# 10XGenomics/vartrix

Hardware: NVIDIA H100
Metric: reads_sw_scored_per_sec (higher is better)
Workload: dtype int16x2

## Files before the change

vartrix_b200/csrc/vtx_sw_fold.cuh:

```cuda
#pragma once
#include <cuda/atomic>
#include "vtx_sw.cuh"
#include "vtx_fold_ring.cuh"

namespace vtx {

constexpr int kFoldP = 96;
constexpr int kFoldC1 = 12;
constexpr int kFoldPPW = 4;
constexpr int kFoldR = 19;
constexpr int kFoldMaxRead = 8 * kFoldR;
constexpr int kFoldMaxMid = 40;
constexpr int kFoldRows = kFoldMaxRead + 4;
constexpr int kFoldCodeStride = kFoldMaxRead + 16;
constexpr int kFoldPairRows = 25;
#ifndef VTX_FOLD_UNROLL
#define VTX_FOLD_UNROLL 4
#endif
constexpr int kFoldDeepWarps = 20, kFoldDeepSlots = 9;
constexpr int kFoldShallowWarps = 13;
#ifndef VTX_FOLD_DEEP_DEPTH
#define VTX_FOLD_DEEP_DEPTH 6
#endif
constexpr uint32_t kFoldDeepDepth = VTX_FOLD_DEEP_DEPTH;
constexpr int kFoldUnroll = VTX_FOLD_UNROLL;
#ifndef VTX_FOLD_MID_UNROLL
#define VTX_FOLD_MID_UNROLL 1
#endif
constexpr int kFoldMidUnroll = VTX_FOLD_MID_UNROLL;

constexpr size_t kFoldSlotBytes = (size_t(kFoldPairRows) * kFoldP + size_t(kFoldMaxMid) * 8) * 4;
constexpr size_t kFoldWarpBytes = size_t(kFoldPPW) * kFoldRows * 8 + 32 + size_t(2 * kFoldPPW) * kFoldCodeStride;
static_assert(kFoldSlotBytes % 16 == 0 && kFoldWarpBytes % 16 == 0, "slots and warp areas stay 16-byte aligned");
template <int S> __host__ __device__ constexpr size_t fold_ring_bytes() { return (sizeof(FoldRing<S>) + 15) & ~size_t(15); }
template <int W, int S> __host__ __device__ constexpr size_t fold_cta_bytes()
{
    return fold_ring_bytes<S>() + S * kFoldSlotBytes + W * kFoldWarpBytes;
}

struct FoldSyncDev {
    using ref = cuda::atomic_ref<uint32_t, cuda::thread_scope_block>;
    __device__ static bool try_lock(uint32_t* p)
    {
        uint32_t z = 0;
        return ref(*p).compare_exchange_strong(z, 1u, cuda::memory_order_acquire, cuda::memory_order_relaxed);
    }
    __device__ static void unlock(uint32_t* p) { ref(*p).store(0u, cuda::memory_order_release); }
    __device__ static uint32_t grab(uint32_t* cursor) { return atomicAdd(cursor, 1u); }
    __device__ static uint32_t load_relaxed(uint32_t* p) { return ref(*p).load(cuda::memory_order_relaxed); }
    __device__ static uint32_t load_acquire(uint32_t* p) { return ref(*p).load(cuda::memory_order_acquire); }
    __device__ static void store_relaxed(uint32_t* p, uint32_t v) { ref(*p).store(v, cuda::memory_order_relaxed); }
    __device__ static void store_release(uint32_t* p, uint32_t v) { ref(*p).store(v, cuda::memory_order_release); }
    __device__ static void add(uint32_t* p, uint32_t v) { ref(*p).fetch_add(v, cuda::memory_order_relaxed); }
    __device__ static void sub_release(uint32_t* p, uint32_t v) { ref(*p).fetch_sub(v, cuda::memory_order_release); }
    __device__ static void pause() { __nanosleep(100); }
};

__device__ __forceinline__ uint32_t fold_locate(const uint32_t* __restrict__ ts, uint32_t n, uint32_t lo, uint32_t t,
                                                int lane)
{
    uint32_t hi = n, step = 1;
    for (;;) {
        const uint32_t i = lo + uint32_t(lane + 1) * step;
        const uint32_t k = __popc(__ballot_sync(0xffffffffu, i < hi && __ldg(ts + i) <= t));
        lo += k * step;
        if (k < 32) hi = min(hi, lo + step);
        if (hi - lo <= 1) return lo;
        step = (hi - lo + 31) / 32;
    }
}

constexpr int kJuncH = -2 * kGoe - kBias, kJuncE = -kGapOpen - kBias;
constexpr uint32_t kJuncH2 = (uint32_t(uint16_t(int16_t(kJuncH - 1))) << 16) | uint32_t(uint16_t(int16_t(kJuncH)));
constexpr uint32_t kJuncE2 = (uint32_t(uint16_t(int16_t(kJuncE - 1))) << 16) | uint32_t(uint16_t(int16_t(kJuncE)));

static_assert(kGapExtend < 0 && kGapOpen <= 0, "the vertical gap is a running maximum only if go <= 0");
constexpr uint32_t kFoldRowY2 = uint32_t(-kGapExtend) * 0x10001u;
constexpr uint32_t kGO2 = pack2(kGapOpen, kGapOpen);
constexpr uint32_t kScanNeg2 = pack2(kBias - 1024, kBias - 1024);
__host__ __device__ constexpr uint32_t fold_row_hg_add(int c)
{
    return (uint32_t(uint16_t(int16_t(kGoe + c * kGapExtend - 1))) << 16) | uint32_t(uint16_t(int16_t(kGoe + c * kGapExtend)));
}
static_assert(fold_row_hg_add(0) == kGoeAdd, "row 0 adds plain goe");

template <int W, int S, bool SHARED>
__global__ void __launch_bounds__(W * 32, 1) vtx_k_sw_fold(const SwArgs a)
{
    constexpr int C1 = kFoldC1, P = kFoldP, R = kFoldR, M = 8;
    constexpr int RS1 = P;

    extern __shared__ __align__(16) uint8_t smem_raw[];
    const int lane = threadIdx.x & 31, warp = threadIdx.x >> 5;
    const int u = lane >> 3, g = lane & 7;
    FoldRing<S>& ring = *reinterpret_cast<FoldRing<S>*>(smem_raw);
    uint8_t* const slots = smem_raw + fold_ring_bytes<S>();
    uint2* bnd = reinterpret_cast<uint2*>(slots + S * kFoldSlotBytes + warp * kFoldWarpBytes);
    uint8_t* codes = reinterpret_cast<uint8_t*>(bnd + kFoldPPW * kFoldRows + 4);

    const uint32_t n_tiles = __ldg(a.tile_start + a.n_loci);
    static_assert(SHARED || S == W, "per-warp tables: one slot per warp");
    const uint32_t run_len = SHARED ? fold_run_len(n_tiles, gridDim.x, W, kTileChunk)
                                    : max(1u, min(uint32_t(kTileChunk), n_tiles / (gridDim.x * W * 16u)));
    const uint32_t one = a.one;
    uint32_t w_next = 0, w_end = 0, w_locus = 0, w_cached = kFoldNoTile;
    if (threadIdx.x == 0) ring_init(ring);
    __syncthreads();

    for (;;) {
        __syncwarp();
        uint32_t tile, locus, slot;
        bool build;
        if constexpr (SHARED) {
            FoldTake tk{};
            if (lane == 0) tk = ring_take<FoldSyncDev>(ring, a.tile_counter, run_len, n_tiles);
            tile = __shfl_sync(0xffffffffu, tk.tile, 0);
            if (tile == kFoldNoTile) break;
            locus = fold_locate(a.tile_start, a.n_loci, __shfl_sync(0xffffffffu, tk.hint, 0), tile, lane);
            FoldBook bk{};
            if (lane == 0) bk = ring_book<FoldSyncDev>(ring, tk.ticket, locus);
            slot = __shfl_sync(0xffffffffu, bk.slot, 0);
            build = __shfl_sync(0xffffffffu, bk.build, 0);
        } else {
            if (w_next == w_end) {
                uint32_t chunk = 0;
                if (lane == 0) chunk = atomicAdd(a.tile_counter, 1u);
                chunk = __shfl_sync(0xffffffffu, chunk, 0);
                w_next = chunk * run_len;
                if (w_next >= n_tiles) break;
                w_end = min(w_next + run_len, n_tiles);
                w_locus = upper_locus(a.tile_start, a.n_loci, w_next);
            }
            tile = w_next++;
            while (tile >= __ldg(a.tile_start + w_locus + 1)) ++w_locus;
            locus = w_locus;
            slot = warp;
            build = locus != w_cached;
            w_cached = locus;
        }
        const uint32_t p0 = __ldg(a.pair_start + locus) + kFoldPPW * (tile - __ldg(a.tile_start + locus));
        const uint32_t p_end = __ldg(a.pair_start + locus + 1);
        uint32_t* prof = reinterpret_cast<uint32_t*>(slots + slot * kFoldSlotBytes);
        uint32_t* midtab = prof + kFoldPairRows * RS1;
        if (build) {
            const uint8_t* rh = a.hap_bytes + __ldg(a.ref_off + locus);
            const uint8_t* ah = a.hap_bytes + __ldg(a.alt_off + locus);
            const int n_ref = int(__ldg(a.ref_len + locus)), n_alt = int(__ldg(a.alt_len + locus));
            const int mid_ref = n_ref - 2 * P, mid_alt = n_alt - 2 * P;
            if (lane == 0) ring.mids[slot] = uint32_t(mid_ref) | uint32_t(mid_alt) << 16;
            if (lane < P / 4) {
                uint32_t fb[4], sb[4];
#pragma unroll
                for (int k = 0; k < 4; ++k) {
                    fb[k] = hap_code(__ldg(rh + 4 * lane + k));
                    sb[k] = hap_code(__ldg(rh + (n_ref - 1 - 4 * lane - k)));
                }
#pragma unroll
                for (uint32_t ra = 0; ra < 5; ++ra)
#pragma unroll
                    for (uint32_t rb = 0; rb < 5; ++rb) {
                        uint32_t w[4];
#pragma unroll
                        for (int k = 0; k < 4; ++k)
                            w[k] = pack2(ra == fb[k] ? kProfMatch : kProfMis, rb == sb[k] ? kProfMatch : kProfMis);
                        reinterpret_cast<uint4*>(prof + (5 * ra + rb) * RS1)[lane] = make_uint4(w[0], w[1], w[2], w[3]);
                    }
            }
            const int lmax = max(mid_ref, mid_alt);
            for (int idx = lane; idx < lmax * 8; idx += 32) {
                const int k = idx >> 3;
                const uint32_t r = uint32_t(idx & 7);
                const uint32_t rb = k < mid_ref ? hap_code(__ldg(rh + P + k)) : 5u;
                const uint32_t ab = k < mid_alt ? hap_code(__ldg(ah + P + k)) : 5u;
                midtab[idx] = pack2(r == rb ? kProfMatch : kProfMis, r == ab ? kProfMatch : kProfMis);
            }
            __syncwarp();
            if (SHARED && lane == 0) ring_publish<FoldSyncDev>(ring, slot);
        } else if (SHARED) {
            ring_wait<FoldSyncDev>(ring, slot);
        }
        const int mid_ref = int(ring.mids[slot] & 0xFFFFu), mid_alt = int(ring.mids[slot] >> 16);
        const uint32_t pair = p0 + u;
        const bool active = pair < p_end;
        int m = 0;
        uint8_t* cf = codes + (2 * u) * kFoldCodeStride;
        uint8_t* cp = cf + kFoldCodeStride;
        {
            const uint8_t* nib = nullptr;
            if (active) {
                const uint32_t rd = __ldg(a.pair_read + pair);
                m = int(__ldg(a.read_len + rd));
                nib = a.read_nib + __ldg(a.read_off + rd);
            }
            for (int e = g; e < kFoldCodeStride; e += 8)
                if (e < M || e >= M + m) cf[e] = 4;
            for (int b = g; 2 * b < m; b += 8) {
                const uint32_t by = __ldg(nib + b);
                cf[M + 2 * b] = uint8_t(nib_code(by >> 4));
                if (2 * b + 1 < m) cf[M + 2 * b + 1] = uint8_t(nib_code(by & 0xF));
            }
            __syncwarp();
            for (int e = g; e < kFoldCodeStride; e += 8)
                cp[e] = (e < M || e >= M + m) ? uint8_t(5 * 4 + 4) : uint8_t(5 * cf[e] + cf[2 * M + m - 1 - e]);
        }
        int mmax = m;
#pragma unroll
        for (int o = 16; o >= 1; o >>= 1) mmax = max(mmax, __shfl_xor_sync(0xffffffffu, mmax, o));
        __syncwarp();

        uint2* my_bnd = bnd + u * kFoldRows;
        const uint2* row_bnd = my_bnd + 7;
        uint32_t best;
        {
            uint32_t hg[C1], f[C1];
#pragma unroll
            for (int c = 0; c < C1; ++c) { hg[c] = kGOE2; f[c] = kNEG2; }
            uint32_t hg_last = kGOE2, e_last = kNEG2, diag_save = kGOE2;
            best = kBIAS2;
            const uint8_t* cA = cp + M - g;
            const uint32_t* lane_p = prof + g * C1;
            const int steps = mmax + 7;
#pragma unroll kFoldUnroll
            for (int t = 0; t < steps; ++t) {
                uint32_t hl = __shfl_up_sync(0xffffffffu, hg_last, 1, 8);
                uint32_t el = __shfl_up_sync(0xffffffffu, e_last, 1, 8);
                if (g == 0) { hl = kGOE2; el = kNEG2; }
                const uint4* pa = reinterpret_cast<const uint4*>(lane_p + uint32_t(cA[t]) * RS1);
                uint32_t diag = diag_save;
                diag_save = hl;
                uint32_t e = el, eg = hl, hleft = hl;
#pragma unroll
                for (int q = 0; q < C1 / 4; ++q) {
                    const uint4 a4 = pa[q];
                    const uint32_t sv[4] = { a4.x, a4.y, a4.z, a4.w };
                    uint32_t hh[4];
#pragma unroll
                    for (int k = 0; k < 4; ++k) {
                        const int c = 4 * q + k;
                        const uint32_t fc = __viaddmax_s16x2(f[c], kGE2, hg[c]);
                        e = __viaddmax_s16x2(e, kGE2, eg);
                        const uint32_t h = sw_h(diag, one, sv[k], fc, e);
                        hh[k] = h;
                        diag = hg[c];
                        hleft = hadd(h, one, c);
                        eg = hleft;
                        hg[c] = hleft;
                        f[c] = fc;
                    }
                    best = __vimax3_s16x2(best, hh[0], hh[1]);
                    best = __vimax3_s16x2(best, hh[2], hh[3]);
                }
                hg_last = hleft;
                e_last = e;
                if (g == 7) my_bnd[t] = make_uint2(hleft, e);
            }
#pragma unroll
            for (int o = 4; o >= 1; o >>= 1) best = __vmaxs2(best, __shfl_xor_sync(0xffffffffu, best, o));
            best = __vmaxs2(best, __byte_perm(best, 0, 0x1032));
        }
        __syncwarp();

        {
            const int lmax = max(mid_ref, mid_alt), lmin = min(mid_ref, mid_alt);
            const uint32_t short_mask = mid_ref < mid_alt ? 0x0000FFFFu : mid_alt < mid_ref ? 0xFFFF0000u : 0u;
            const int k_short = lmin != lmax ? lmin - 1 : -1;
            uint32_t hg[R], e[R], rc[R];
            const uint8_t* cfm = cf + M + R * g;
#pragma unroll
            for (int c = 0; c < R; ++c) {
                const int row = R * g + c;
                uint2 b = make_uint2(kGOE2, kNEG2);
                if (row < mmax) b = row_bnd[row];
                hg[c] = __byte_perm(b.x, 0, 0x1010);
                e[c] = __byte_perm(b.y, 0, 0x1010);
                rc[c] = uint32_t(cfm[c]) * 4u;
            }
            const int jlim = m - 2 - R * g;
            const uint2* jbnd = row_bnd + jlim;
            auto junction = [&](uint32_t mask) {
                uint32_t cross = kBIAS2;
#pragma unroll
                for (int c = 0; c < R; ++c) {
                    uint2 b = make_uint2(kGOE2, kGOE2);
                    if (c <= jlim) b = jbnd[-c];
                    const uint32_t ph = __byte_perm(b.x, 0, 0x3232), pe = __byte_perm(b.y, 0, 0x3232);
                    const uint32_t x1 = hg[c] + ph + kJuncH2;
                    const uint32_t x2 = e[c] + pe + kJuncE2;
                    cross = __vimax3_s16x2(cross, x1, x2);
                }
                best = __vmaxs2(best, (cross & mask) | (kBIAS2 & ~mask));
            };
            const uint8_t* tab = reinterpret_cast<const uint8_t*>(midtab);
#pragma unroll kFoldMidUnroll
            for (int k = 0; k < lmax; ++k) {
                const uint8_t* trow = tab + 32 * k;
                uint32_t diag = __shfl_up_sync(0xffffffffu, hg[R - 1], 1, 8);
                if (g == 0) diag = kGOE2;
                uint32_t aa[2], yy[2], ymax = kBIAS2;
#pragma unroll
                for (int c = 0; c < R; ++c) {
                    const uint32_t sv = *reinterpret_cast<const uint32_t*>(trow + rc[c]);
                    const uint32_t ec = __viaddmax_s16x2(e[c], kGE2, hg[c]);
                    const uint32_t av = __vimax3_s16x2(diag + sv, ec, kBIAS2);
                    const uint32_t yv = av + kFoldRowY2 * uint32_t(c);
                    diag = hg[c];
                    hg[c] = yv;
                    e[c] = ec;
                    aa[c & 1] = av;
                    yy[c & 1] = yv;
                    if (c & 1) {
                        best = __vimax3_s16x2(best, aa[0], aa[1]);
                        ymax = __vimax3_s16x2(ymax, yy[0], yy[1]);
                    }
                }
                if (R & 1) {
                    best = __vmaxs2(best, aa[0]);
                    ymax = __vmaxs2(ymax, yy[0]);
                }
                const uint32_t lane_ofs = uint32_t(-kGapExtend * R * g) * 0x10001u;
                uint32_t p = __shfl_up_sync(0xffffffffu, ymax + lane_ofs, 1, 8);
                if (g == 0) p = kScanNeg2;
#pragma unroll
                for (int o = 1; o < 8; o <<= 1) p = __vmaxs2(p, __shfl_up_sync(0xffffffffu, p, o, 8));
                p -= lane_ofs;
#pragma unroll
                for (int c = 0; c < R; ++c) {
                    const uint32_t yv = hg[c];
                    hg[c] = __viaddmax_s16x2(p, kGO2, yv) + fold_row_hg_add(c);
                    if (c + 1 < R) p = __vmaxs2(p, yv);
                }
                if (k == k_short) junction(short_mask);
            }
            junction(~short_mask);
#pragma unroll
            for (int o = 4; o >= 1; o >>= 1) best = __vmaxs2(best, __shfl_xor_sync(0xffffffffu, best, o));
            __syncwarp();
            if (SHARED && lane == 0) ring_release<FoldSyncDev>(ring, slot);
            if (active && g == 0) call_and_scatter(a, pair, best - kBIAS2);
        }
    }
}

}
```

Baseline: 169.5 million.

## Extend fold through shared mid-haplotype prefix before splitting ref/alt lanes

Detects how many middle haplotype bases ref and alt share at both ends and builds per-column 25-entry pair profiles for them. The kernel then runs those shared columns in a fused forward/backward mode before switching into the existing ref/alt split, shortening the split loop and junction span. The intent is to reduce the per-read column work in the middle region, at the cost of extra build logic, a parked boundary write to shared memory, and a repacked mids encoding limited to 8-bit lengths.

```diff
diff --git a/vartrix_b200/csrc/vtx_sw_fold.cuh b/vartrix_b200/csrc/vtx_sw_fold.cuh
--- a/vartrix_b200/csrc/vtx_sw_fold.cuh
+++ b/vartrix_b200/csrc/vtx_sw_fold.cuh
@@ -29,7 +29,8 @@
 #endif
 constexpr int kFoldMidUnroll = VTX_FOLD_MID_UNROLL;
 
-constexpr size_t kFoldSlotBytes = (size_t(kFoldPairRows) * kFoldP + size_t(kFoldMaxMid) * 8) * 4;
+constexpr int kFoldMidTabBytes = kFoldMaxMid * 32, kFoldExtColBytes = kFoldPairRows * 4;
+constexpr size_t kFoldSlotBytes = size_t(kFoldPairRows) * kFoldP * 4 + kFoldMidTabBytes;
 constexpr size_t kFoldWarpBytes = size_t(kFoldPPW) * kFoldRows * 8 + 32 + size_t(2 * kFoldPPW) * kFoldCodeStride;
 static_assert(kFoldSlotBytes % 16 == 0 && kFoldWarpBytes % 16 == 0, "slots and warp areas stay 16-byte aligned");
 template <int S> __host__ __device__ constexpr size_t fold_ring_bytes() { return (sizeof(FoldRing<S>) + 15) & ~size_t(15); }
@@ -147,7 +148,6 @@
             const uint8_t* ah = a.hap_bytes + __ldg(a.alt_off + locus);
             const int n_ref = int(__ldg(a.ref_len + locus)), n_alt = int(__ldg(a.alt_len + locus));
             const int mid_ref = n_ref - 2 * P, mid_alt = n_alt - 2 * P;
-            if (lane == 0) ring.mids[slot] = uint32_t(mid_ref) | uint32_t(mid_alt) << 16;
             if (lane < P / 4) {
                 uint32_t fb[4], sb[4];
 #pragma unroll
@@ -166,20 +166,34 @@
                         reinterpret_cast<uint4*>(prof + (5 * ra + rb) * RS1)[lane] = make_uint4(w[0], w[1], w[2], w[3]);
                     }
             }
-            const int lmax = max(mid_ref, mid_alt);
-            for (int idx = lane; idx < lmax * 8; idx += 32) {
+            const int lmax = max(mid_ref, mid_alt), lmin = min(mid_ref, mid_alt);
+            const int x_cap = min((lmin - 1) / 2, (kFoldMidTabBytes - 32 * lmax) / (kFoldExtColBytes - 64));
+            const bool shared = lane < x_cap && __ldg(rh + P + lane) == __ldg(ah + P + lane) &&
+                                __ldg(rh + (n_ref - 1 - P - lane)) == __ldg(ah + (n_alt - 1 - P - lane));
+            const int x = __ffs(~__ballot_sync(0xffffffffu, shared)) - 1;
+            const int am_ref = mid_ref - 2 * x, am_alt = mid_alt - 2 * x;
+            if (lane == 0) ring.mids[slot] = uint32_t(am_ref) | uint32_t(am_alt) << 8 | uint32_t(x) << 16;
+            if (lane < x) {
+                const uint32_t fb = hap_code(__ldg(rh + P + lane)), sb = hap_code(__ldg(rh + (n_ref - 1 - P - lane)));
+#pragma unroll
+                for (uint32_t ra = 0; ra < 5; ++ra)
+#pragma unroll
+                    for (uint32_t rb = 0; rb < 5; ++rb)
+                        midtab[lane * kFoldPairRows + 5 * ra + rb] = pack2(ra == fb ? kProfMatch : kProfMis, rb == sb ? kProfMatch : kProfMis);
+            }
+            uint32_t* alltab = midtab + x * kFoldPairRows;
+            for (int idx = lane; idx < (lmax - 2 * x) * 8; idx += 32) {
                 const int k = idx >> 3;
                 const uint32_t r = uint32_t(idx & 7);
-                const uint32_t rb = k < mid_ref ? hap_code(__ldg(rh + P + k)) : 5u;
-                const uint32_t ab = k < mid_alt ? hap_code(__ldg(ah + P + k)) : 5u;
-                midtab[idx] = pack2(r == rb ? kProfMatch : kProfMis, r == ab ? kProfMatch : kProfMis);
+                const uint32_t rb = k < am_ref ? hap_code(__ldg(rh + P + x + k)) : 5u;
+                const uint32_t ab = k < am_alt ? hap_code(__ldg(ah + P + x + k)) : 5u;
+                alltab[idx] = pack2(r == rb ? kProfMatch : kProfMis, r == ab ? kProfMatch : kProfMis);
             }
             __syncwarp();
             if (SHARED && lane == 0) ring_publish<FoldSyncDev>(ring, slot);
         } else if (SHARED) {
             ring_wait<FoldSyncDev>(ring, slot);
         }
-        const int mid_ref = int(ring.mids[slot] & 0xFFFFu), mid_alt = int(ring.mids[slot] >> 16);
         const uint32_t pair = p0 + u;
         const bool active = pair < p_end;
         int m = 0;
@@ -261,19 +275,18 @@
         __syncwarp();
 
         {
-            const int lmax = max(mid_ref, mid_alt), lmin = min(mid_ref, mid_alt);
-            const uint32_t short_mask = mid_ref < mid_alt ? 0x0000FFFFu : mid_alt < mid_ref ? 0xFFFF0000u : 0u;
-            const int k_short = lmin != lmax ? lmin - 1 : -1;
+            const uint32_t mids = ring.mids[slot];
             uint32_t hg[R], e[R], rc[R];
+            const uint8_t* cpm = cp + M + R * g;
             const uint8_t* cfm = cf + M + R * g;
 #pragma unroll
             for (int c = 0; c < R; ++c) {
                 const int row = R * g + c;
                 uint2 b = make_uint2(kGOE2, kNEG2);
                 if (row < mmax) b = row_bnd[row];
-                hg[c] = __byte_perm(b.x, 0, 0x1010);
-                e[c] = __byte_perm(b.y, 0, 0x1010);
-                rc[c] = uint32_t(cfm[c]) * 4u;
+                hg[c] = b.x;
+                e[c] = b.y;
+                rc[c] = uint32_t(cpm[c]) * 4u;
             }
             const int jlim = m - 2 - R * g;
             const uint2* jbnd = row_bnd + jlim;
@@ -290,10 +303,7 @@
                 }
                 best = __vmaxs2(best, (cross & mask) | (kBIAS2 & ~mask));
             };
-            const uint8_t* tab = reinterpret_cast<const uint8_t*>(midtab);
-#pragma unroll kFoldMidUnroll
-            for (int k = 0; k < lmax; ++k) {
-                const uint8_t* trow = tab + 32 * k;
+            auto column = [&](const uint8_t* trow) {
                 uint32_t diag = __shfl_up_sync(0xffffffffu, hg[R - 1], 1, 8);
                 if (g == 0) diag = kGOE2;
                 uint32_t aa[2], yy[2], ymax = kBIAS2;
@@ -329,6 +339,26 @@
                     hg[c] = __viaddmax_s16x2(p, kGO2, yv) + fold_row_hg_add(c);
                     if (c + 1 < R) p = __vmaxs2(p, yv);
                 }
+            };
+            const uint8_t* tab = reinterpret_cast<const uint8_t*>(midtab);
+            for (int k = int(mids >> 16); k > 0; --k, tab += kFoldExtColBytes) column(tab);
+            best = __vmaxs2(best, __byte_perm(best, 0, 0x1032));
+            uint2* park = my_bnd + 7 + R * g;
+#pragma unroll
+            for (int c = 0; c < R; ++c) {
+                park[c] = make_uint2(hg[c], e[c]);
+                hg[c] = __byte_perm(hg[c], 0, 0x1010);
+                e[c] = __byte_perm(e[c], 0, 0x1010);
+                rc[c] = uint32_t(cfm[c]) * 4u;
+            }
+            __syncwarp();
+            const int mid_ref = int(mids & 0xFFu), mid_alt = int((mids >> 8) & 0xFFu);
+            const int lmax = max(mid_ref, mid_alt), lmin = min(mid_ref, mid_alt);
+            const uint32_t short_mask = mid_ref < mid_alt ? 0x0000FFFFu : mid_alt < mid_ref ? 0xFFFF0000u : 0u;
+            const int k_short = lmin != lmax ? lmin - 1 : -1;
+#pragma unroll kFoldMidUnroll
+            for (int k = 0; k < lmax; ++k) {
+                column(tab + 32 * k);
                 if (k == k_short) junction(short_mask);
             }
             junction(~short_mask);
```

Result: faster. 176.8 million, median of 6 (+4.3%).
